# LiangZhaoPKUImperial/LinearSFM

Hardware: AMD Instinct MI355X
Metric: hierarchical linear map-joining solve wall-clock, NC3500-like stereo (all transforms + joins) (lower is better)
Workload: dtype f64

## Files before the change

### include/lsfm.h

```cpp
#ifndef LSFM_H
#define LSFM_H

#include <stddef.h>

#ifdef __cplusplus
extern "C" {
#endif

#define LSFM_OK 0
#define LSFM_ERR_ARG (-1)
#define LSFM_ERR_NO_DEVICE (-2)
#define LSFM_ERR_HIP (-3)
#define LSFM_ERR_OOM (-4)
#define LSFM_ERR_INTERNAL (-5)
#define LSFM_ERR_IO (-6)
#define LSFM_ERR_NOT_SPD (-7)
#define LSFM_NOT_CONVERGED 1

typedef struct lsfm_context lsfm_context;

typedef struct lsfm_map {
	int Ref, FRef, m, n, nU, nW;
	int ScaP, Fix, Sign, FScaP, FFix;
	int* stno;
// ... 170 lines not shown
int lsfm_save_pair_gate(const char* path, const int* ids, int K, const double* d2, const double* cov_diff);
int lsfm_read_pair_gate(const char* path, int* ids_f, int* ids_g, double* d2, double* cov_diff, int cap, int* count);
int lsfm_save_merge_report(const char* path, int K, int removed, int dof, double d2, const int* ids);
int lsfm_read_merge_report(const char* path, int* K, int* removed, int* dof, double* d2, int* ids, int cap);
int lsfm_save_state(const char* path, const double* st, const int* stno, int n);
int lsfm_save_state_bin(const char* path, const double* st, const int* stno, int n);
int lsfm_save_poses(const char* pose_path, const char* feat_path, const int* stno, const double* st, int n);

int lsfm_spmv_bench(lsfm_context* ctx, int m, const int* rowptr, const int* colidx, const double* val,
                    const double* x, double* y, int reps, double* avg_ms, double* algorithmic_bytes);

int lsfm_wstream_bench(lsfm_context* ctx, long long nblocks, int mode, int reps, double* avg_ms);

int lsfm_selftest_prims(lsfm_context* ctx, int cases, unsigned seed);

#define LSFM_SELFTEST_CHOL_INFO 16
int lsfm_selftest_chol(lsfm_context* ctx, int m, const int* rowptr, const int* colidx, const double* val, const int* origin, const unsigned char* fixed,
                       const int* pose_seg, int nseg, const double* r, int nrhs, int mode, double* z, double* dot, int* perm, int* colptr, int* rowidx,
                       double* L, double* Dinv, double* dscale, int cap_blocks, int* info);

int lsfm_selftest_transform(lsfm_context* ctx, const lsfm_map* maps, int N, int mono, const int* tref, const int* tscap, const int* tfix,
                            int alias_passthrough, lsfm_map* out);

int lsfm_selftest_small(lsfm_context* ctx, int G, const int* pose_off, const int* feat_off, const int* u_off, const unsigned char* active,
                        const double* U, const int* Ui, const int* Uj, const double* W, const int* photo, const int* feature, int nW, const double* V,
                        const double* ea, const double* eb, const double* x0, const unsigned char* fixed, int strips, double* x_pose, double* x_feat,
                        int* status, double* max_rel);

#ifdef __cplusplus
}
// ... 3 lines not shown
```

### linearsfm_amd/api.py

```python
from __future__ import annotations

import ctypes as C
import os

import numpy as np

_HERE = os.path.dirname(os.path.abspath(__file__))
LIB_PATH = os.path.join(_HERE, "liblsfm_hip.so")
_LIB = None

LSFM_OK = 0
LSFM_NOT_CONVERGED = 1


class LsfmMap(C.Structure):
    _fields_ = [("Ref", C.c_int), ("FRef", C.c_int), ("m", C.c_int), ("n", C.c_int), ("nU", C.c_int), ("nW", C.c_int),
                ("ScaP", C.c_int), ("Fix", C.c_int), ("Sign", C.c_int), ("FScaP", C.c_int), ("FFix", C.c_int),
                ("stno", C.POINTER(C.c_int)), ("stVal", C.POINTER(C.c_double)),
                ("U", C.POINTER(C.c_double)), ("Ui", C.POINTER(C.c_int)), ("Uj", C.POINTER(C.c_int)),
                ("W", C.POINTER(C.c_double)), ("photo", C.POINTER(C.c_int)), ("feature", C.POINTER(C.c_int)),
                ("V", C.POINTER(C.c_double)), ("FBlock", C.POINTER(C.c_int)), ("pose_origin", C.POINTER(C.c_int))]


class LsfmStats(C.Structure):
# ... 72 lines not shown
        L.lsfm_tree_free.argtypes = [vp, vp]
        L.lsfm_tree_free.restype = None
        L.lsfm_divide_conquer.argtypes = [vp, P(LsfmMap), C.c_int, C.c_int, P(LsfmMap), P(LsfmStats)]
        L.lsfm_read_localmap.argtypes = [C.c_char_p, C.c_int, P(LsfmMap)]
        L.lsfm_write_localmap.argtypes = [C.c_char_p, C.c_int, P(LsfmMap)]
        L.lsfm_read_localmaps.argtypes = [C.c_char_p, C.c_int, C.c_int, C.c_int, C.c_int, P(LsfmMap), P(C.c_int)]
        L.lsfm_write_mapset.argtypes = [C.c_char_p, P(LsfmMap), C.c_int, C.c_int]
        L.lsfm_mapset_info.argtypes = [C.c_char_p, P(C.c_int), P(C.c_int)]
        L.lsfm_read_mapset.argtypes = [C.c_char_p, C.c_int, C.c_int, C.c_int, C.c_int, P(LsfmMap)]
        L.lsfm_save_state_bin.argtypes = [C.c_char_p, P(C.c_double), P(C.c_int), C.c_int]
        L.lsfm_save_state.argtypes = [C.c_char_p, dp, ip, C.c_int]
        L.lsfm_save_poses.argtypes = [C.c_char_p, C.c_char_p, ip, dp, C.c_int]
        L.lsfm_schur_pattern.argtypes = [vp, ip, ip, ip, ip, C.c_int, C.c_int, C.c_int, C.c_int, ip, ip, C.c_int, ip]
        L.lsfm_symbolic_analyse.argtypes = [C.c_int, ip, ip, ip, C.c_int, ip, ip, ip, C.c_int, ip, dp]
        L.lsfm_inverse_v.argtypes = [vp, dp, C.c_int, C.c_int]
        L.lsfm_gn_polish.argtypes = [vp, P(LsfmMap), C.c_int, C.c_int, P(LsfmMap), C.c_int, dp, dp, ip]
        L.lsfm_gn_polish_robust.argtypes = [vp, P(LsfmMap), C.c_int, C.c_int, P(LsfmMap), C.c_int, C.c_int, C.c_double, dp, dp, ip, dp, dp]
        L.lsfm_map_chi2.argtypes = [vp, P(LsfmMap), C.c_int, C.c_int, P(LsfmMap), dp, ip]
        L.lsfm_map_feature_chi2.argtypes = [vp, P(LsfmMap), C.c_int, C.c_int, P(LsfmMap), dp, dp]
        L.lsfm_gn_polish_robust_features.argtypes = [vp, P(LsfmMap), C.c_int, C.c_int, P(LsfmMap), C.c_int, C.c_int, C.c_double, dp, dp, ip, dp, dp]
        L.lsfm_gn_linearise.argtypes = [vp, P(LsfmMap), C.c_int, C.c_int, P(LsfmMap), dp, P(LsfmMap), dp, dp]
        L.lsfm_gn_linearise_timed.argtypes = [vp, P(LsfmMap), C.c_int, C.c_int, P(LsfmMap), dp, P(LsfmMap), dp, dp, dp, ip]
        L.lsfm_solve_features.argtypes = [vp, dp, dp, dp, dp, dp, dp, C.c_int, C.c_int, ip, ip]
        L.lsfm_map_covariance.argtypes = [vp, P(LsfmMap), C.c_int, dp, dp, dp, C.c_int, ip]
        L.lsfm_map_covariance_timed.argtypes = [vp, P(LsfmMap), C.c_int, dp, dp, dp, C.c_int, ip, dp]
        L.lsfm_save_covariances.argtypes = [C.c_char_p, C.c_char_p, ip, C.c_int, C.c_int, dp, dp]
        L.lsfm_read_covariances.argtypes = [C.c_char_p, C.c_int, ip, dp, C.c_int, ip]
        L.lsfm_map_covariance_columns.argtypes = [vp, P(LsfmMap), C.c_int, ip, C.c_int, dp, dp, dp, ip, dp]
        L.lsfm_map_covariance_columns_timed.argtypes = [vp, P(LsfmMap), C.c_int, ip, C.c_int, dp, dp, dp, ip, dp, dp]
        L.lsfm_map_covariance_feature_columns.argtypes = [vp, P(LsfmMap), C.c_int, ip, C.c_int, dp, dp, dp, ip, dp]
# ... 26 lines not shown
        L.lsfm_selftest_chol.argtypes = [vp, C.c_int, ip, ip, dp, ip, P(C.c_ubyte), ip, C.c_int, dp, C.c_int, C.c_int, dp, dp, ip, ip, ip, dp, dp, dp,
                                         C.c_int, ip]
        L.lsfm_selftest_transform.argtypes = [vp, P(LsfmMap), C.c_int, C.c_int, ip, ip, ip, C.c_int, P(LsfmMap)]
        L.lsfm_selftest_small.argtypes = [vp, C.c_int, ip, ip, ip, ub, dp, ip, ip, dp, ip, ip, C.c_int, dp, dp, dp, dp, ub, C.c_int, dp, dp, ip, dp]
        _LIB = L
    return _LIB


EXPORTS = ["lsfm_context_create", "lsfm_context_destroy", "lsfm_set_pcg", "lsfm_set_precision", "lsfm_set_small_solve", "lsfm_set_spmv_variant", "lsfm_set_covcols_panel", "lsfm_last_error", "lsfm_stream",
           "lsfm_map_release", "lsfm_transform_stereo", "lsfm_transform_mono", "lsfm_join_stereo", "lsfm_join_mono",
           "lsfm_solve_stereo", "lsfm_solve_mono", "lsfm_tree_upload", "lsfm_tree_run", "lsfm_tree_set_final_reanchor",
           "lsfm_tree_download", "lsfm_tree_set_stop_level", "lsfm_tree_node_count", "lsfm_tree_download_node", "lsfm_tree_download_state", "lsfm_tree_set_plans", "lsfm_tree_export_size", "lsfm_tree_export_dev", "lsfm_packed_size",
           "lsfm_tree_upload_dev", "lsfm_tree_reload_dev", "lsfm_tree_set_comm", "lsfm_tree_set_comm_blocks", "lsfm_tree_export_slice_sizes", "lsfm_tree_export_slice_dev",
           "lsfm_tree_free", "lsfm_divide_conquer", "lsfm_read_localmap", "lsfm_read_localmaps", "lsfm_write_localmap", "lsfm_write_mapset", "lsfm_mapset_info", "lsfm_mapset_stamp", "lsfm_read_mapset", "lsfm_save_state_bin", "lsfm_save_state", "lsfm_save_poses", "lsfm_gn_polish",
           "lsfm_gn_polish_robust", "lsfm_map_chi2", "lsfm_map_feature_chi2", "lsfm_gn_polish_robust_features", "lsfm_gn_linearise", "lsfm_gn_linearise_timed",
           "lsfm_spmv_bench", "lsfm_wstream_bench", "lsfm_selftest_prims", "lsfm_selftest_chol", "lsfm_selftest_transform", "lsfm_selftest_small", "lsfm_schur_pattern", "lsfm_symbolic_analyse", "lsfm_inverse_v", "lsfm_solve_features",
           "lsfm_map_covariance", "lsfm_map_covariance_timed",
           "lsfm_save_covariances", "lsfm_read_covariances",
           "lsfm_map_covariance_columns", "lsfm_map_covariance_columns_timed", "lsfm_save_cov_columns", "lsfm_read_cov_columns",
           "lsfm_map_covariance_feature_columns", "lsfm_map_covariance_feature_columns_timed", "lsfm_map_feature_pair_gate", "lsfm_map_feature_pair_gate_timed", "lsfm_save_pair_gate", "lsfm_read_pair_gate",
           "lsfm_map_merge_features", "lsfm_map_merge_features_timed", "lsfm_merge_structure", "lsfm_save_merge_report", "lsfm_read_merge_report",
           "lsfm_map_marginalise", "lsfm_map_marginalise_timed", "lsfm_tree_export_reduced_size", "lsfm_tree_export_reduced_dev",
           "lsfm_tree_export_reduced_dev_timed", "lsfm_map_marginalise_poses", "lsfm_map_marginalise_poses_timed", "lsfm_marg_pose_structure", "lsfm_gn_structure"]


def _c(a, dtype):
    return np.ascontiguousarray(a, dtype=dtype).reshape(-1)


def _ptr(a, ctype):
    return a.ctypes.data_as(C.POINTER(ctype))
# ... 311 lines not shown
        t, cnt = np.zeros(3), np.zeros(4, np.int32)
        rc = lib().lsfm_gn_linearise_timed(self._h, arr, len(hms), int(mono), C.byref(x), _ptr(w, C.c_double) if w is not None else None,
                                           C.byref(out), C.byref(F), _ptr(b, C.c_double) if want_b else None,
                                           _ptr(t, C.c_double) if timed else None, _ptr(cnt, C.c_int) if timed else None)
        self._check(rc, "lsfm_gn_linearise")
        d = map_to_dict(out)
        if timed:
            return d, F.value, b, dict(zip(("assembly_ms", "coalesce_w_ms", "coalesce_u_ms"), t.tolist())), dict(zip(("NWJ", "nW", "NUJ", "nU"), cnt.tolist()))
        return d, F.value, b

    def inverse_v(self, V):
        IV = np.array(np.asarray(V, np.float64).reshape(-1), copy=True)
        n = IV.size // 9
        self._check(lib().lsfm_inverse_v(self._h, _ptr(IV, C.c_double), 0, n), "lsfm_inverse_v")
        return IV.reshape(n, 9)

    def solve_features(self, j, IV, eb, dpa):
        m, n = int(j["m"]), int(j["n"])
        W = _c(j["W"], np.float64); ph = _c(j["photo"], np.int32); fe = _c(j["feature"], np.int32)
        cnt = np.bincount(fe, minlength=n).astype(np.int32)
        IV = _c(IV, np.float64); eb = _c(eb, np.float64); dpa = _c(dpa, np.float64)
        dpb = np.zeros(3 * n)
        self._check(lib().lsfm_solve_features(self._h, _ptr(W, C.c_double), _ptr(IV, C.c_double), None, _ptr(eb, C.c_double), _ptr(dpa, C.c_double),
                                              _ptr(dpb, C.c_double), m, n, _ptr(cnt, C.c_int), _ptr(ph, C.c_int)), "lsfm_solve_features")
        return dpb

    def schur_pattern(self, j):
        m, n = int(j["m"]), int(j["n"])
        Ui = _c(j["Ui"], np.int32); Uj = _c(j["Uj"], np.int32); ph = _c(j["photo"], np.int32); fe = _c(j["feature"], np.int32)
        cap = m * (m + 1) // 2
# ... 526 lines not shown
```

### linearsfm_amd/csrc/lsfm_capi.hip

```cpp
#include <climits>
#include <cmath>
#include <cstring>

#include "lsfm_internal.hpp"
#include "lsfm_marg.hpp"
#include "lsfm_solve.hpp"
#include "lsfm_system.hpp"
#include "lsfm_tree.hpp"

using namespace lsfm;

namespace {

template <class F> int guarded(lsfm_context* ctx, F&& f)
{
	if (!ctx) return LSFM_ERR_ARG;
	struct Reset {
		lsfm_context* c;
		~Reset() { c->timed.clear(); c->ev_next = 0; c->plan = nullptr; }
	} reset{ ctx };
	try
	{
		if (hipSetDevice(ctx->device) != hipSuccess) return LSFM_ERR_NO_DEVICE;
		return f();
// ... 585 lines not shown
}

int lsfm_map_merge_features(lsfm_context* ctx, const lsfm_map* map, int mono, const int* pairs, int K, lsfm_map* out, double* d2, int* dof, int* rep,
                            int* steps, double* last_corr)
{
	return lsfm_map_merge_features_timed(ctx, map, mono, pairs, K, out, d2, dof, rep, steps, last_corr, nullptr);
}

int lsfm_inverse_v(lsfm_context* ctx, double* V, int m, int n)
{
	(void)m;
	if (n < 0 || (n && !V)) return LSFM_ERR_ARG;
	return guarded(ctx, [&]() { return inverse_v(ctx, V, n); });
}

int lsfm_solve_features(lsfm_context* ctx, const double* W, const double* IV, const double* ea, const double* eb, const double* dpa, double* dpb,
                        int m, int n, const int* mapCor, const int* photo)
{
	(void)ea;
	if (m <= 0 || n < 0 || !dpa || (n && (!W || !IV || !eb || !dpb || !mapCor || !photo))) return LSFM_ERR_ARG;
	return guarded(ctx, [&]() { return solve_features(ctx, W, IV, eb, dpa, dpb, m, n, mapCor, photo); });
}

int lsfm_schur_pattern(lsfm_context* ctx, const int* Ui, const int* Uj, const int* photo, const int* feature, int m, int n, int nU, int nW, int* rowptr,
                       int* colidx, int cap, int* nnzb)
{
	if (m <= 0 || n < 0 || nU < 0 || nW < 0 || !rowptr || !colidx || !nnzb || (nU && (!Ui || !Uj)) || (nW && (!photo || !feature))) return LSFM_ERR_ARG;
	return guarded(ctx, [&]() {
		HostSystem h;
		h.m = m; h.n = n; h.nU = nU; h.nW = nW;
// ... 107 lines not shown
```

### linearsfm_amd/csrc/lsfm_device.hpp

```cpp
#pragma once
#include <hip/hip_runtime.h>

#define LSFM_WAVE 64
#define LSFM_PI_REF 3.1415926

namespace lsfm {

__device__ __forceinline__ bool tr_stereo_hub(int pose_id, int tref) { return tref >= 0 && pose_id == tref; }
__device__ __forceinline__ bool tr_keeps_u(int a, int b, int h0, int h1) { return a != h0 && b != h0 && a != h1 && b != h1; }
__device__ __forceinline__ bool tr_keeps_w(int k, int h0, int h1) { return k != h0 && k != h1; }

template <int N>
__device__ __forceinline__ void ld(double* dst, const double* __restrict__ src)
{
#pragma unroll
	for (int i = 0; i < N; i++) dst[i] = src[i];
}
template <int N>
__device__ __forceinline__ void ld(double* dst, const float* __restrict__ src)
{
#pragma unroll
	for (int i = 0; i < N; i++) dst[i] = (double)src[i];
}
template <int N>
// ... 159 lines not shown
	for (int off = 32; off > 0; off >>= 1) v += __shfl_xor(v, off, LSFM_WAVE);
	return v;
}
template <int LANES>
__device__ __forceinline__ double block_sum_fixed(double v, double* part)
{
	v = wave_sum(v);
	if ((threadIdx.x & (LSFM_WAVE - 1)) == 0) part[threadIdx.x / LSFM_WAVE] = v;
	__syncthreads();
	double sum = 0.0;
#pragma unroll
	for (int w = 0; w < LANES / LSFM_WAVE; w++) sum += part[w];
	return sum;
}

__device__ __forceinline__ void atomic_add_f64(double* p, double v)
{
	__hip_atomic_fetch_add(p, v, __ATOMIC_RELAXED, __HIP_MEMORY_SCOPE_AGENT);
}

__device__ __forceinline__ void atomic_add_i64(long long* p, long long v)
{
	__hip_atomic_fetch_add(reinterpret_cast<unsigned long long*>(p), (unsigned long long)v, __ATOMIC_RELAXED, __HIP_MEMORY_SCOPE_AGENT);
}
__device__ __forceinline__ void lds_add_i64(long long* p, long long v)
{
	__hip_atomic_fetch_add(reinterpret_cast<unsigned long long*>(p), (unsigned long long)v, __ATOMIC_RELAXED, __HIP_MEMORY_SCOPE_WORKGROUP);
}
__device__ __forceinline__ long long to_fixed(double v, int sh, bool& bad)
{
// ... 105 lines not shown
	if (!valid) return;
	const int sl = lds_slot(keys, cap, key);
#pragma unroll
	for (int i = 0; i < N; i++) stage[i] = x[i];
	const int rot = (threadIdx.x & (LSFM_WAVE - 1)) % N;
#pragma unroll 1
	for (int e = 0; e < N; e++)
	{
		int i = e + rot;
		if (i >= N) i -= N;
		const double v = stage[i];
		if (sl >= 0) lds_add_f64(vals + sl * N + i, v); else atomic_add_f64(gdst + i, v);
	}
}
template <int N>
__device__ __forceinline__ void tile_clear(int* keys, double* vals, int cap)
{
	for (int i = threadIdx.x; i < cap; i += blockDim.x) keys[i] = -1;
	for (int i = threadIdx.x; i < cap * N; i += blockDim.x) vals[i] = 0.0;
}
template <int N>
__device__ __forceinline__ void tile_flush(const int* keys, const double* vals, int cap, double* gbase)
{
	for (int i = threadIdx.x; i < cap * N; i += blockDim.x)
	{
		const int k = keys[i / N];
		if (k >= 0) atomic_add_f64(gbase + (size_t)k * N + i % N, vals[i]);
	}
}

template <int TW, class EntryFn, class FeatFn>
__device__ __forceinline__ void tile_runs(int nft, const int* sFp, double* sT, EntryFn entry, FeatFn feat)
{
	const int tid = threadIdx.x, nt = blockDim.x;
	int la = 0;
	while (la < nft)
	{
		const int e0 = sFp[la];
		int lo = la + 1, hi = nft;
		while (lo < hi) { const int mid = (lo + hi + 1) >> 1; if (sFp[mid] - e0 <= nt) lo = mid; else hi = mid - 1; }
		const int lb = lo, e1 = sFp[lb];
		for (int ce0 = e0;; ce0 += nt)
		{
// ... 26 lines not shown
```

### linearsfm_amd/csrc/lsfm_internal.hpp

```cpp
#pragma once
#include <hip/hip_runtime.h>

#include <cstdint>
#include <cstdio>
#include <condition_variable>
#include <cstring>
#include <exception>
#include <functional>
#include <memory>
#include <mutex>
#include <thread>
#include <string>
#include <vector>

#include "../../include/lsfm.h"
#include "lsfm_map.hpp"

namespace lsfm {

struct Error { int code; std::string msg; };
struct DevBatch;
struct IndexHold;
struct SolvePlan;
struct PreLevel;
// ... 379 lines not shown
                       int* halvings, double* fchi2, double* fweight);
int map_chi2(lsfm_context* ctx, const lsfm_map* maps, int N, bool mono, const lsfm_map* x, double* chi2, int* dof);
int gn_linearise(lsfm_context* ctx, const lsfm_map* maps, int N, bool mono, const lsfm_map* x, const double* weight, lsfm_map* out, double* obj,
                 double* b, double* times, int* counts);
int map_covariance(lsfm_context* ctx, const lsfm_map* map, bool mono, double* pose_cov, double* feat_cov, double* pair_cov, int cap_blocks, int* nnzb,
                   double* times);
int map_covariance_columns(lsfm_context* ctx, const lsfm_map* map, bool mono, const int* poses, int k, double* pose_cols, double* feat_cols, double* joint,
                           int* steps, double* last_corr, double* times);
int map_covariance_feature_columns(lsfm_context* ctx, const lsfm_map* map, bool mono, const int* feats, int k, double* pose_cols, double* feat_cols,
                                   double* joint, int* steps, double* last_corr, double* times);
int map_feature_pair_gate(lsfm_context* ctx, const lsfm_map* map, bool mono, const int* pairs, int K, double* d2, double* cov_diff, int* steps,
                          double* last_corr, double* times);
int map_merge_features(lsfm_context* ctx, const lsfm_map* map, bool mono, const int* pairs, int K, lsfm_map* out, double* d2, int* dof, int* rep,
                       int* steps, double* last_corr, double* times);
int inverse_v(lsfm_context* ctx, double* V, int n);
int solve_features(lsfm_context* ctx, const double* W, const double* IV, const double* eb, const double* dpa, double* dpb, int m, int n, const int* mapCor,
                   const int* photo);
bool no_timing_events();
#define LSFM_REC_T(e, s) do { if (!lsfm::no_timing_events()) LSFM_CHECK_HIP(hipEventRecord(e, s)); } while (0)
unsigned timing_event_flags();
unsigned order_event_flags();
void prefetch_next_level(lsfm_context* ctx, const DevBatch& Y, const std::vector<int>& target_ref, int next_level, int step_hint,
                         const unsigned long long* level_keys, int level_nnzb);
int spmv_external(lsfm_context* ctx, int m, const int* rowptr, const int* colidx, const double* val, const double* x, double* y, int reps,
                  double* avg_ms, double* bytes);
int chol_selftest(lsfm_context* ctx, int m, const int* rowptr, const int* colidx, const double* val, const int* origin, const unsigned char* fixed,
                  const int* pose_seg, int nseg, const double* r, int nrhs, int mode, double* z, double* dot, int* perm, int* colptr, int* rowidx,
                  double* L, double* Dinv, double* dscale, int cap_blocks, int* info);

int wstream_bench(lsfm_context* ctx, long long nblocks, int mode, int reps, double* avg_ms);
// ... 3 lines not shown
```

### linearsfm_amd/csrc/lsfm_solve.hip

```cpp
#include <algorithm>
#include <cmath>

#include "lsfm_device.hpp"
#include "lsfm_internal.hpp"
#include "lsfm_solve.hpp"

namespace lsfm {

__global__ void __launch_bounds__(256) k_vinv(int NF, const double* __restrict__ V, const double* __restrict__ eb, double* __restrict__ IV, double* __restrict__ LY,
                                               double* __restrict__ ymax, RhsFused rhs, double* __restrict__ uu)
{
	__shared__ double wmax[4];
	int f = blockIdx.x * blockDim.x + threadIdx.x;
	double y2 = 0.0;
	if (f < NF)
	{
	double a[9], o[9];
	ld<9>(a, V + (size_t)f * 9);
	inv3_sym(a, o);
	st<9>(IV + (size_t)f * 9, o);
	const double* e = eb + (size_t)f * 3;
	double l[9];
	const double d0 = o[0];
	l[0] = sqrt(d0);
	l[1] = o[3] / l[0];
	l[3] = o[6] / l[0];
	const double d1 = o[4] - l[1] * l[1];
	l[2] = sqrt(d1);
	l[4] = (o[7] - l[3] * l[1]) / l[2];
	const double d2 = o[8] - l[3] * l[3] - l[4] * l[4];
	l[5] = sqrt(d2);
	l[6] = l[0] * e[0] + l[1] * e[1] + l[3] * e[2];
	l[7] = l[2] * e[1] + l[4] * e[2];
	l[8] = l[5] * e[2];
	if (!(d0 > 0.0) || !(d1 > 0.0) || !(d2 > 0.0)) l[0] = __builtin_nan("");
	st<9>(LY + (size_t)f * 9, l);
	y2 = l[6] * l[6] + l[7] * l[7] + l[8] * l[8];
	if (uu)
	{
#pragma unroll
		for (int sd = 0; sd < 2; sd++)
		{
			const int fs = sd ? rhs.srcC[f] : rhs.srcE[f];
			double u0 = 0.0, u1 = 0.0, u2 = 0.0;
			if (fs >= 0)
			{
				const double* x = rhs.feat_src + (size_t)fs * 3;
				u0 = x[0] / l[0];
				u1 = (x[1] - l[1] * u0) / l[2];
				u2 = (x[2] - l[3] * u0 - l[4] * u1) / l[5];
			}
			uu[(size_t)f * 6 + 3 * sd] = u0; uu[(size_t)f * 6 + 3 * sd + 1] = u1; uu[(size_t)f * 6 + 3 * sd + 2] = u2;
			y2 = fmax(y2, u0 * u0 + u1 * u1 + u2 * u2);
		}
	}
	if (!(y2 == y2)) y2 = 0.0;
	}
	if (!ymax) return;
#pragma unroll
	for (int off = 32; off > 0; off >>= 1) y2 = fmax(y2, __shfl_xor(y2, off, LSFM_WAVE));
	if ((threadIdx.x & (LSFM_WAVE - 1)) == 0) wmax[threadIdx.x >> 6] = y2;
	__syncthreads();
	if (threadIdx.x == 0) ymax[blockIdx.x] = fmax(fmax(wmax[0], wmax[1]), fmax(wmax[2], wmax[3]));
}

__device__ __forceinline__ int half_exponent(double d)
{
	if (!(d > 0.0) || !(d < 1e300)) return 0;
	int k;
	(void)frexp(d, &k);
	return ((k + 1) >> 1) + 1;
}
// ... 652 lines not shown
{
	ctx->ensure_arenas((size_t)n * 400 + ((size_t)64 << 20));
	ctx->arena[0].reset(); ctx->scratch.reset();
	double* dV = ctx->arena[0].alloc<double>((size_t)n * 9);
	double* dIV = ctx->arena[0].alloc<double>((size_t)n * 9);
	h2d(ctx, dV, V, (size_t)n * 9 * sizeof(double));
	if (n)
	{
		double* LY = ctx->scratch.alloc<double>((size_t)n * 9);
		double* eb = ctx->scratch.alloc<double>((size_t)n * 3);
		dev_zero(ctx, eb, (size_t)n * 3 * sizeof(double));
		hipLaunchKernelGGL(k_vinv, dim3((n + 255) / 256), dim3(256), 0, ctx->stream, n, dV, eb, dIV, LY, (double*)nullptr, RhsFused(), (double*)nullptr);
		LSFM_CHECK_HIP(hipStreamSynchronize(ctx->stream));
	}
	d2h(ctx, V, dIV, (size_t)n * 9 * sizeof(double));
	return LSFM_OK;
}
int solve_features(lsfm_context* ctx, const double* W, const double* IV, const double* eb, const double* dpa, double* dpb, int m, int n, const int* mapCor,
                   const int* photo)
{
	std::vector<int> fptr((size_t)n + 1, 0);
	for (int f = 0; f < n; f++)
	{
		if (mapCor[f] < 0) LSFM_FAIL(LSFM_ERR_ARG, "negative block count of a feature");
		fptr[f + 1] = fptr[f] + mapCor[f];
	}
	const int nW = fptr[n];
	for (int j = 0; j < nW; j++) if (photo[j] < 0 || photo[j] >= m) LSFM_FAIL(LSFM_ERR_ARG, "photo index out of range");
	ctx->ensure_arenas((size_t)nW * 200 + (size_t)n * 300 + (size_t)m * 100 + ((size_t)64 << 20));
	ctx->arena[0].reset(); ctx->scratch.reset();
// ... 56 lines not shown
```

### linearsfm_amd/csrc/lsfm_transform.hip

```cpp
#include <algorithm>
#include <climits>
#include <cstddef>

#include "lsfm_device.hpp"
#include "lsfm_internal.hpp"

namespace lsfm {

struct TMap {
	int active, nh;
	int P0, m, F0, n;
	int U0, U0n, W0, W0n, kU0, kW0;
	int hub[2];
	int nref, nscap;
	int newFix, oldFix, newLabel;
	int c2fix, c3zero;
	int tref, tscap, oldref, oldscap;
	double R1[9], t1[3], scale1;
	int sign1;
	double R[9], dRA[9], dRB[9], dRG[9], t[3], dA[3], dB[3], dG[3];
	double Scale, Scale2, dSdA[3], dSdB[3], dSdG[3], dSdt[9], dSdtt[9];
};

__global__ void k_tr_find(const int* __restrict__ pose_id, const int* __restrict__ pose_map, int M, TMap* tm)
// ... 258 lines not shown

__global__ void k_tr_gather_counts(const int* __restrict__ KU, const int* __restrict__ KW, const int* __restrict__ uoff, const int* __restrict__ woff,
                                   int B, int* __restrict__ out, const TMap* __restrict__ tm, const int* __restrict__ err)
{
	int b = blockIdx.x * blockDim.x + threadIdx.x;
	if (b > B) return;
	out[b] = KU[uoff[b]];
	out[B + 1 + b] = KW[woff[b]];
	if (b < B) out[2 * (B + 1) + b] = tm[b].active > 0 ? tm[b].sign1 : 0;
	else out[2 * (B + 1) + B] = *err;
}

#define TRE_TILE 128
#define TRE_ROUND 256
#define TRE_MAPS 4
#define TR_REC 39
static_assert(offsetof(TMap, dRA) == offsetof(TMap, R) + 72 && offsetof(TMap, dRB) == offsetof(TMap, R) + 144 && offsetof(TMap, dRG) == offsetof(TMap, R) + 216 &&
              offsetof(TMap, t) == offsetof(TMap, R) + 288, "R, dRA, dRB, dRG, t of TMap are read as one run of TR_REC doubles");

__device__ __forceinline__ void stereo_tf(const double* rec, const double* xn, double* Tf)
{
	double dd[3] = { xn[0] - rec[36], xn[1] - rec[37], xn[2] - rec[38] }, tmp1[3], tmp2[3], tmp3[3];
	mv3(rec + 9, dd, tmp1); mv3(rec + 18, dd, tmp2); mv3(rec + 27, dd, tmp3);
#pragma unroll
	for (int r = 0; r < 3; r++) { Tf[3 * r] = tmp1[r]; Tf[3 * r + 1] = tmp2[r]; Tf[3 * r + 2] = tmp3[r]; }
}

template <int NH>
__global__ void __launch_bounds__(256)
k_tr_feat_pre(int NF, const TMap* __restrict__ tm, const int* __restrict__ feat_map, const double* __restrict__ feat, const int* __restrict__ fptr,
              const double* __restrict__ Vold, const int* __restrict__ KW, double* __restrict__ nfeat, int* __restrict__ nfptr,
              double* __restrict__ Vn, double* __restrict__ FD, int4* __restrict__ finfo, int* __restrict__ hubJ)
{
	const int f = blockIdx.x * blockDim.x + threadIdx.x;
	if (f >= NF) return;
#pragma unroll
	for (int sidx = 0; sidx < NH; sidx++) hubJ[(size_t)f * NH + sidx] = -1;
	const TMap* t = &tm[feat_map[f]];
	const int j0 = fptr[f];
	const double* x = feat + (size_t)f * 3;
	if (!(t->active > 0 && t->nh == NH))
	{
		nfeat[3 * (size_t)f] = x[0]; nfeat[3 * (size_t)f + 1] = x[1]; nfeat[3 * (size_t)f + 2] = x[2];
		for (int i = 0; i < 9; i++) Vn[(size_t)f * 9 + i] = Vold[(size_t)f * 9 + i];
		nfptr[f] = t->W0n + (j0 - t->W0);
		finfo[f] = make_int4(0, -1, NH == 2 ? -1 : feat_map[f], -j0);
		return;
	}
	nfptr[f] = t->W0n + NH * (f - t->F0) + (KW[j0] - t->kW0);
	finfo[f] = make_int4(1, t->hub[0], NH == 2 ? t->hub[1] : feat_map[f], NH - KW[j0]);
	double Df[9], Cf[NH][18], xn[3];
	double d[3] = { x[0] - t->t1[0], x[1] - t->t1[1], x[2] - t->t1[2] };
	mv3(t->R1, d, xn);
	if (NH == 2) { xn[0] = xn[0] / t->scale1; xn[1] = xn[1] / t->scale1; xn[2] = xn[2] / t->scale1; }
	nfeat[3 * (size_t)f] = xn[0]; nfeat[3 * (size_t)f + 1] = xn[1]; nfeat[3 * (size_t)f + 2] = xn[2];
	if constexpr (NH == 1)
	{
		ld<9>(Df, t->R);
	}
	else
	{
		double adt[9], atmp[9], adtt[9];
		mono_trans_jac(*t, xn, Df, adt, atmp, adtt);
#pragma unroll
		for (int r = 0; r < 3; r++)
		{
#pragma unroll
			for (int c = 0; c < 3; c++) { Cf[0][6 * r + c] = adt[3 * r + c]; Cf[NH - 1][6 * r + c] = adtt[3 * r + c]; Cf[NH - 1][6 * r + 3 + c] = 0.0; }
			Cf[0][6 * r + 3] = atmp[3 * r]; Cf[0][6 * r + 4] = atmp[3 * r + 1]; Cf[0][6 * r + 5] = atmp[3 * r + 2];
		}
		if (t->c2fix)
#pragma unroll
			for (int r = 0; r < 3; r++)
#pragma unroll
				for (int c = 0; c < 6; c++)
					if (c == t->newFix) Cf[0][6 * r + c] = 0.0;
		if (t->c3zero) zero<18>(Cf[NH - 1]);
	}
	double V[9], T[9], Vnew[9];
	ld<9>(V, Vold + (size_t)f * 9);
	mtm<3, 3, 3, false>(Df, V, T);
	mm<3, 3, 3, false>(T, Df, Vnew);
	st<9>(Vn + (size_t)f * 9, Vnew);
	if constexpr (NH == 2)
	{
		double* fd = FD + (size_t)f * (9 + 18 * NH);
		st<9>(fd, Df);
#pragma unroll
		for (int s = 0; s < NH; s++) st<18>(fd + 9 + 18 * s, Cf[s]);
	}
}

#ifdef LSFM_K9_TIMING
__device__ unsigned long long g_tr_t[16];
#define TRT_DECL unsigned long long tracc[12] = { 0, 0, 0, 0, 0, 0, 0, 0, 0, 0, 0, 0 }; unsigned long long trprev = __builtin_readcyclecounter()
#define TRT(i) do { const unsigned long long n_ = __builtin_readcyclecounter(); tracc[i] += n_ - trprev; trprev = n_; } while (0)
#define TRT_FLUSH() do { if (threadIdx.x == 0) { for (int i_ = 0; i_ < 12; i_++) atomicAdd(&g_tr_t[i_], tracc[i_]); atomicAdd(&g_tr_t[12], 1ull); } } while (0)
extern "C" void lsfm_debug_tr(unsigned long long* out, int reset)
{
	(void)hipDeviceSynchronize();
	if (out) (void)hipMemcpyFromSymbol(out, HIP_SYMBOL(g_tr_t), sizeof(unsigned long long) * 16);
	if (reset) { unsigned long long z[16] = { 0 }; (void)hipMemcpyToSymbol(HIP_SYMBOL(g_tr_t), z, sizeof(z)); }
}
#else
#define TRT_DECL do { } while (0)
// ... 288 lines not shown
#pragma unroll
	for (int s = 0; s < NH; s++) tile_flush<36>(gkeys, gvals + s * GCAP * 36, GCAP, Gpose + (size_t)s * M * 36);
	TRT(9);
	TRT_FLUSH();
}

template <int NH>
__global__ void __launch_bounds__(256, NH == 1 ? 2 : 1)
k_tr_feat_post(int NF, int M, const TMap* __restrict__ tm, const int* __restrict__ feat_map, const int* __restrict__ fptr,
               const double* __restrict__ Vold, const double* __restrict__ Wold, const int* __restrict__ photo, const double* __restrict__ Dp,
               const double* __restrict__ FD, const double* __restrict__ xnew, const double* __restrict__ Gsum, const int* __restrict__ hubJ,
               const int* __restrict__ wbase, const int* __restrict__ newf, int* __restrict__ srcf, double* __restrict__ Wn_,
               int* __restrict__ nphoto, int* __restrict__ nfeature, double* __restrict__ PP)
{
	constexpr int TW = 18 * NH;
	const int f = blockIdx.x * blockDim.x + threadIdx.x;
	const bool inb = f < NF;
	const TMap* t = inb ? &tm[feat_map[f]] : nullptr;
	const bool act = inb && t->active > 0 && t->nh == NH;
	double Df[9], Cf[NH][18], G[NH][18];
	if (act)
	{
		const double* fd = NH == 2 ? FD + (size_t)f * (9 + TW) : nullptr;
		if constexpr (NH == 1) ld<9>(Df, t->R); else ld<9>(Df, fd);
		const int base = wbase[f];
		const int hubs[2] = { t->hub[0], NH == 2 ? t->hub[1] : -1 };
		double hubW[NH][18];
#pragma unroll
		for (int s = 0; s < NH; s++) zero<18>(hubW[s]);
		bool walk = false;
// ... 54 lines not shown
			mtm<3, 6, 3, true>(G[s], Df, Wh);
			st<18>(Wn_ + (size_t)(base + s) * 18, Wh);
			nphoto[base + s] = hubs[s]; nfeature[base + s] = newf ? newf[f] : f;
			if (srcf) srcf[base + s] = f;
		}
	}
#pragma unroll
	for (int s = 0; s < NH; s++)
#pragma unroll
		for (int s2 = s; s2 < NH; s2++)
		{
			double P[36];
			if (act) mtm<3, 6, 6, false>(Cf[s], G[s2], P);
			const int idx = (s == 0 ? s2 : 2);
			const int mp = act ? feat_map[f] : 0;
			wave_scatter_add<36>(PP + ((size_t)mp * 3 + idx) * 36, P, act);
		}
}

template <int NH>
__global__ void __launch_bounds__(128, 1)
k_tr_ublocks(int NU, int M, const TMap* __restrict__ tm, const int* __restrict__ pose_map, const double* __restrict__ Uold,
             const int* __restrict__ Ui, const int* __restrict__ Uj, const int* __restrict__ KU, const double* __restrict__ Dp,
             const double* __restrict__ Cp, double* __restrict__ Un, int* __restrict__ nUi, int* __restrict__ nUj,
             double* __restrict__ Gpose)
{
	constexpr int GCAP = 64;
	__shared__ int gkeys[GCAP];
	__shared__ double gvals[NH * GCAP * 36];
	__shared__ double sStage[128 * 37];
	for (int q = threadIdx.x; q < GCAP; q += blockDim.x) gkeys[q] = -1;
	for (int q = threadIdx.x; q < NH * GCAP * 36; q += blockDim.x) gvals[q] = 0.0;
// ... 65 lines not shown
}

__device__ __forceinline__ void add_oriented(double* dst, const double* X, int r, int c)
{
	if (r < c) { for (int q = 0; q < 36; q++) dst[q] += X[q]; }
	else if (r > c) { for (int i = 0; i < 6; i++) for (int j = 0; j < 6; j++) dst[j * 6 + i] += X[i * 6 + j]; }
	else { for (int i = 0; i < 6; i++) for (int j = 0; j < 6; j++) dst[i * 6 + j] += X[i * 6 + j] + X[j * 6 + i]; }
}

template <int NH>
__global__ void __launch_bounds__(128, 1)
k_tr_poseslots(int M, const TMap* __restrict__ tm, const int* __restrict__ pose_map, const double* __restrict__ Dp,
                               const double* __restrict__ Cp, const double* __restrict__ Gpose, double* __restrict__ Un, int* __restrict__ nUi,
                               int* __restrict__ nUj, double* __restrict__ PP)
{
	const int k0 = blockIdx.x * blockDim.x + threadIdx.x;
	const bool inb = k0 < M;
	const int k = inb ? k0 : 0;
	const int mp = pose_map[k];
	const TMap& t = tm[mp];
	const bool act = inb && t.active > 0 && t.nh == NH;
	double D[36];
	ld<36>(D, Dp + (size_t)k * 36);
	const int h0 = t.hub[0], h1 = NH == 2 ? t.hub[1] : -1;
	const int slot1 = t.U0n + (k - t.P0), slot2 = t.U0n + t.m + (k - t.P0);
	if (act)
	{
		if (k <= h0) { nUi[slot1] = k; nUj[slot1] = h0; } else { nUi[slot1] = h0; nUj[slot1] = k; }
		if (NH == 2) { if (k <= h0) { nUi[slot2] = k; nUj[slot2] = h1; } else { nUi[slot2] = h1; nUj[slot2] = k; } }
	}
// ... 11 lines not shown
			if (h0 < h1) { for (int q = 0; q < 36; q++) atomic_add_f64(dst + q, X[q]); }
			else { for (int i = 0; i < 6; i++) for (int j = 0; j < 6; j++) atomic_add_f64(dst + j * 6 + i, X[i * 6 + j]); }
		}
		else if (NH == 2 && s == 0 && k == h1)
		{
			double* dst = Un + (size_t)slot1 * 36;
			if (h1 < h0) { for (int q = 0; q < 36; q++) atomic_add_f64(dst + q, X[q]); }
			else { for (int i = 0; i < 6; i++) for (int j = 0; j < 6; j++) atomic_add_f64(dst + j * 6 + i, X[i * 6 + j]); }
		}
		else
		{
			double* dst = Un + (size_t)(s == 0 ? slot1 : slot2) * 36;
			add_oriented(dst, X, k, hs);
		}
#pragma unroll
		for (int s0 = 0; s0 <= s; s0++)
		{
			double C[36], P[36];
			ld<36>(C, Cp + (size_t)s0 * M * 36 + (size_t)k * 36);
			mtm<6, 6, 6, false>(C, G, P);
			const int idx = (s0 == 0 ? s : 2);
			wave_scatter_add<36>(PP + ((size_t)mp * 3 + idx) * 36, P, act);
		}
	}
}

template <int NH>
__global__ void k_tr_diag(int B, const TMap* __restrict__ tm, const double* __restrict__ PP, double* __restrict__ Un)
{
	int b = blockIdx.x * blockDim.x + threadIdx.x;
	if (b >= B) return;
	const TMap& t = tm[b];
	if (t.active <= 0 || t.nh != NH) return;
	const double* P = PP + (size_t)b * 3 * 36;
	double* d0 = Un + (size_t)(t.U0n + (t.hub[0] - t.P0)) * 36;
	for (int q = 0; q < 36; q++) d0[q] += P[q];
	if (NH == 2)
	{
		double* d2 = Un + (size_t)(t.U0n + t.m + (t.hub[1] - t.P0)) * 36;
// ... 301 lines not shown
```

Before: 30.52.

## Stage strided feature records through LDS and tile per-map projection accumulation

Routes the per-feature 9- and 3-double records in k_vinv and k_tr_feat_pre through shared-memory tiles, so global loads and stores become coalesced double2 accesses instead of strided per-thread ones. Replaces wave_scatter_add on the per-map PP accumulators with a new wave-level segmented reduction into a small LDS hash tile, flushed once per block, to cut global f64 atomics. The cost is more shared memory, extra barriers, and a wave shuffle reduction tree. A self-test entry point for the inverse-V kernel is also added.

```diff
diff --git a/include/lsfm.h b/include/lsfm.h
--- a/include/lsfm.h
+++ b/include/lsfm.h
@@ -208,6 +208,8 @@
 
 int lsfm_selftest_prims(lsfm_context* ctx, int cases, unsigned seed);
 
+int lsfm_selftest_vinv(lsfm_context* ctx, const double* V, const double* eb, int n, int skip, double* IV, double* LY);
+
 #define LSFM_SELFTEST_CHOL_INFO 16
 int lsfm_selftest_chol(lsfm_context* ctx, int m, const int* rowptr, const int* colidx, const double* val, const int* origin, const unsigned char* fixed,
                        const int* pose_seg, int nseg, const double* r, int nrhs, int mode, double* z, double* dot, int* perm, int* colptr, int* rowidx,
diff --git a/linearsfm_amd/api.py b/linearsfm_amd/api.py
--- a/linearsfm_amd/api.py
+++ b/linearsfm_amd/api.py
@@ -110,6 +110,7 @@
         L.lsfm_schur_pattern.argtypes = [vp, ip, ip, ip, ip, C.c_int, C.c_int, C.c_int, C.c_int, ip, ip, C.c_int, ip]
         L.lsfm_symbolic_analyse.argtypes = [C.c_int, ip, ip, ip, C.c_int, ip, ip, ip, C.c_int, ip, dp]
         L.lsfm_inverse_v.argtypes = [vp, dp, C.c_int, C.c_int]
+        L.lsfm_selftest_vinv.argtypes = [vp, dp, dp, C.c_int, C.c_int, dp, dp]
         L.lsfm_gn_polish.argtypes = [vp, P(LsfmMap), C.c_int, C.c_int, P(LsfmMap), C.c_int, dp, dp, ip]
         L.lsfm_gn_polish_robust.argtypes = [vp, P(LsfmMap), C.c_int, C.c_int, P(LsfmMap), C.c_int, C.c_int, C.c_double, dp, dp, ip, dp, dp]
         L.lsfm_map_chi2.argtypes = [vp, P(LsfmMap), C.c_int, C.c_int, P(LsfmMap), dp, ip]
@@ -166,7 +167,7 @@
            "lsfm_tree_upload_dev", "lsfm_tree_reload_dev", "lsfm_tree_set_comm", "lsfm_tree_set_comm_blocks", "lsfm_tree_export_slice_sizes", "lsfm_tree_export_slice_dev",
            "lsfm_tree_free", "lsfm_divide_conquer", "lsfm_read_localmap", "lsfm_read_localmaps", "lsfm_write_localmap", "lsfm_write_mapset", "lsfm_mapset_info", "lsfm_mapset_stamp", "lsfm_read_mapset", "lsfm_save_state_bin", "lsfm_save_state", "lsfm_save_poses", "lsfm_gn_polish",
            "lsfm_gn_polish_robust", "lsfm_map_chi2", "lsfm_map_feature_chi2", "lsfm_gn_polish_robust_features", "lsfm_gn_linearise", "lsfm_gn_linearise_timed",
-           "lsfm_spmv_bench", "lsfm_wstream_bench", "lsfm_selftest_prims", "lsfm_selftest_chol", "lsfm_selftest_transform", "lsfm_selftest_small", "lsfm_schur_pattern", "lsfm_symbolic_analyse", "lsfm_inverse_v", "lsfm_solve_features",
+           "lsfm_spmv_bench", "lsfm_wstream_bench", "lsfm_selftest_prims", "lsfm_selftest_chol", "lsfm_selftest_transform", "lsfm_selftest_small", "lsfm_schur_pattern", "lsfm_symbolic_analyse", "lsfm_inverse_v", "lsfm_selftest_vinv", "lsfm_solve_features",
            "lsfm_map_covariance", "lsfm_map_covariance_timed",
            "lsfm_save_covariances", "lsfm_read_covariances",
            "lsfm_map_covariance_columns", "lsfm_map_covariance_columns_timed", "lsfm_save_cov_columns", "lsfm_read_cov_columns",
@@ -508,6 +509,16 @@
         n = IV.size // 9
         self._check(lib().lsfm_inverse_v(self._h, _ptr(IV, C.c_double), 0, n), "lsfm_inverse_v")
         return IV.reshape(n, 9)
+
+    def selftest_vinv(self, V, eb, skip=0):
+        V = _c(np.asarray(V, np.float64).reshape(-1), np.float64); eb = _c(np.asarray(eb, np.float64).reshape(-1), np.float64)
+        n = V.size // 9
+        if V.size != 9 * n or eb.size != 3 * n:
+            raise LsfmError("selftest_vinv: V [n, 9] and eb [n, 3]")
+        IV = np.zeros(9 * n); LY = np.zeros(9 * n)
+        self._check(lib().lsfm_selftest_vinv(self._h, _ptr(V, C.c_double), _ptr(eb, C.c_double), n, int(skip), _ptr(IV, C.c_double), _ptr(LY, C.c_double)),
+                    "lsfm_selftest_vinv")
+        return IV.reshape(n, 9), LY.reshape(n, 9)
 
     def solve_features(self, j, IV, eb, dpa):
         m, n = int(j["m"]), int(j["n"])
diff --git a/linearsfm_amd/csrc/lsfm_capi.hip b/linearsfm_amd/csrc/lsfm_capi.hip
--- a/linearsfm_amd/csrc/lsfm_capi.hip
+++ b/linearsfm_amd/csrc/lsfm_capi.hip
@@ -623,6 +623,12 @@
 	return guarded(ctx, [&]() { return inverse_v(ctx, V, n); });
 }
 
+int lsfm_selftest_vinv(lsfm_context* ctx, const double* V, const double* eb, int n, int skip, double* IV, double* LY)
+{
+	if (n < 0 || skip < 0 || skip > 1 || (n && (!V || !eb || !IV || !LY))) return LSFM_ERR_ARG;
+	return guarded(ctx, [&]() { return vinv_selftest(ctx, V, eb, n, skip, IV, LY); });
+}
+
 int lsfm_solve_features(lsfm_context* ctx, const double* W, const double* IV, const double* ea, const double* eb, const double* dpa, double* dpb,
                         int m, int n, const int* mapCor, const int* photo)
 {
diff --git a/linearsfm_amd/csrc/lsfm_device.hpp b/linearsfm_amd/csrc/lsfm_device.hpp
--- a/linearsfm_amd/csrc/lsfm_device.hpp
+++ b/linearsfm_amd/csrc/lsfm_device.hpp
@@ -197,6 +197,38 @@
 	return sum;
 }
 
+template <int S, int OFF>
+__device__ __forceinline__ double wave_sum_spread(const double* v, bool on, int lane)
+{
+	if constexpr (OFF == 0) return on ? v[0] : 0.0;
+	else
+	{
+		constexpr int H = (S + 1) / 2;
+		const bool up = (lane & OFF) != 0;
+		double w[H];
+#pragma unroll
+		for (int i = 0; i < H; i++)
+		{
+			const double lo = on ? v[i] : 0.0, hi = (i + H < S && on) ? v[i + H < S ? i + H : 0] : 0.0;
+			w[i] = (up ? hi : lo) + __shfl_xor(up ? lo : hi, OFF, LSFM_WAVE);
+		}
+		return wave_sum_spread<H, OFF / 2>(w, true, lane);
+	}
+}
+template <int S>
+__device__ __forceinline__ int wave_spread_index(int lane)
+{
+	int off = 0, len = S, s = S;
+#pragma unroll
+	for (int o = LSFM_WAVE / 2; o; o >>= 1)
+	{
+		const int h = (s + 1) / 2;
+		if (lane & o) { off += h; len -= h; } else len = min(len, h);
+		s = h;
+	}
+	return len >= 1 ? off : -1;
+}
+
 __device__ __forceinline__ void atomic_add_f64(double* p, double v)
 {
 	__hip_atomic_fetch_add(p, v, __ATOMIC_RELAXED, __HIP_MEMORY_SCOPE_AGENT);
@@ -332,6 +364,39 @@
 	}
 }
 template <int N>
+__device__ __forceinline__ void tile_wave_add(int* keys, double* vals, int cap, int key, double* gbase, const double* x, bool valid)
+{
+	static_assert(N <= LSFM_WAVE, "one lane per value");
+	unsigned long long todo = __ballot(valid), alone = 0ull;
+	if (todo == 0ull) return;
+	const int lane = threadIdx.x & (LSFM_WAVE - 1), mine = wave_spread_index<N>(lane);
+#pragma unroll 1
+	for (int round = 0; round < 4 && todo; round++)
+	{
+		const int leader = __ffsll((long long)todo) - 1;
+		const int first = __shfl(key, leader, LSFM_WAVE);
+		const bool same = valid && key == first;
+		const unsigned long long grp = __ballot(same);
+		if (__popcll(grp) > 1)
+		{
+			const double keep = wave_sum_spread<N, LSFM_WAVE / 2>(x, same, lane);
+			int sl = -1;
+			if (lane == leader) sl = lds_slot(keys, cap, first);
+			sl = __shfl(sl, leader, LSFM_WAVE);
+			if (mine >= 0) { if (sl >= 0) lds_add_f64(vals + sl * N + mine, keep); else atomic_add_f64(gbase + (size_t)first * N + mine, keep); }
+		}
+		else alone |= grp;
+		todo &= ~grp;
+	}
+	alone |= todo;
+	if (valid && ((alone >> lane) & 1ull))
+	{
+		const int sl = lds_slot(keys, cap, key);
+#pragma unroll
+		for (int i = 0; i < N; i++) { if (sl >= 0) lds_add_f64(vals + sl * N + i, x[i]); else atomic_add_f64(gbase + (size_t)key * N + i, x[i]); }
+	}
+}
+template <int N>
 __device__ __forceinline__ void tile_clear(int* keys, double* vals, int cap)
 {
 	for (int i = threadIdx.x; i < cap; i += blockDim.x) keys[i] = -1;
@@ -345,6 +410,38 @@
 		const int k = keys[i / N];
 		if (k >= 0) atomic_add_f64(gbase + (size_t)k * N + i % N, vals[i]);
 	}
+}
+
+template <int N>
+__device__ __forceinline__ void tile_records_load(double* tile, const double* __restrict__ g, int nrec)
+{
+	static_assert(N % 2 == 1, "an even record length needs a padded stride in the tile");
+	const int len = nrec * N, head = (int)(((size_t)g >> 3) & 1);
+	if (len <= 0) return;
+	if (threadIdx.x == 0 && head) tile[0] = g[0];
+	const int pairs = (len - head) >> 1;
+	for (int p = threadIdx.x; p < pairs; p += blockDim.x)
+	{
+		const int j = head + 2 * p;
+		const double2 v = *reinterpret_cast<const double2*>(g + j);
+		tile[j] = v.x; tile[j + 1] = v.y;
+	}
+	if (threadIdx.x == 0 && ((len - head) & 1)) tile[len - 1] = g[len - 1];
+}
+template <int N>
+__device__ __forceinline__ void tile_records_store(const double* tile, double* __restrict__ g, int nrec)
+{
+	static_assert(N % 2 == 1, "an even record length needs a padded stride in the tile");
+	const int len = nrec * N, head = (int)(((size_t)g >> 3) & 1);
+	if (len <= 0) return;
+	if (threadIdx.x == 0 && head) g[0] = tile[0];
+	const int pairs = (len - head) >> 1;
+	for (int p = threadIdx.x; p < pairs; p += blockDim.x)
+	{
+		const int j = head + 2 * p;
+		*reinterpret_cast<double2*>(g + j) = make_double2(tile[j], tile[j + 1]);
+	}
+	if (threadIdx.x == 0 && ((len - head) & 1)) g[len - 1] = tile[len - 1];
 }
 
 template <int TW, class EntryFn, class FeatFn>
diff --git a/linearsfm_amd/csrc/lsfm_internal.hpp b/linearsfm_amd/csrc/lsfm_internal.hpp
--- a/linearsfm_amd/csrc/lsfm_internal.hpp
+++ b/linearsfm_amd/csrc/lsfm_internal.hpp
@@ -417,6 +417,7 @@
 int map_merge_features(lsfm_context* ctx, const lsfm_map* map, bool mono, const int* pairs, int K, lsfm_map* out, double* d2, int* dof, int* rep,
                        int* steps, double* last_corr, double* times);
 int inverse_v(lsfm_context* ctx, double* V, int n);
+int vinv_selftest(lsfm_context* ctx, const double* V, const double* eb, int n, int skip, double* IV, double* LY);
 int solve_features(lsfm_context* ctx, const double* W, const double* IV, const double* eb, const double* dpa, double* dpb, int m, int n, const int* mapCor,
                    const int* photo);
 bool no_timing_events();
diff --git a/linearsfm_amd/csrc/lsfm_solve.hip b/linearsfm_amd/csrc/lsfm_solve.hip
--- a/linearsfm_amd/csrc/lsfm_solve.hip
+++ b/linearsfm_amd/csrc/lsfm_solve.hip
@@ -11,16 +11,22 @@
                                                double* __restrict__ ymax, RhsFused rhs, double* __restrict__ uu)
 {
 	__shared__ double wmax[4];
-	int f = blockIdx.x * blockDim.x + threadIdx.x;
+	__shared__ double sRec[256 * 9], sEb[256 * 3];
+	const int f0 = blockIdx.x * 256, nrec = min(256, NF - f0);
+	int f = f0 + threadIdx.x;
+	tile_records_load<9>(sRec, V + (size_t)f0 * 9, nrec);
+	tile_records_load<3>(sEb, eb + (size_t)f0 * 3, nrec);
+	__syncthreads();
 	double y2 = 0.0;
+	double* rec = sRec + threadIdx.x * 9;
+	double l[9];
 	if (f < NF)
 	{
 	double a[9], o[9];
-	ld<9>(a, V + (size_t)f * 9);
+	ld<9>(a, rec);
 	inv3_sym(a, o);
-	st<9>(IV + (size_t)f * 9, o);
-	const double* e = eb + (size_t)f * 3;
-	double l[9];
+	st<9>(rec, o);
+	const double* e = sEb + threadIdx.x * 3;
 	const double d0 = o[0];
 	l[0] = sqrt(d0);
 	l[1] = o[3] / l[0];
@@ -34,7 +40,6 @@
 	l[7] = l[2] * e[1] + l[4] * e[2];
 	l[8] = l[5] * e[2];
 	if (!(d0 > 0.0) || !(d1 > 0.0) || !(d2 > 0.0)) l[0] = __builtin_nan("");
-	st<9>(LY + (size_t)f * 9, l);
 	y2 = l[6] * l[6] + l[7] * l[7] + l[8] * l[8];
 	if (uu)
 	{
@@ -56,6 +61,12 @@
 	}
 	if (!(y2 == y2)) y2 = 0.0;
 	}
+	__syncthreads();
+	tile_records_store<9>(sRec, IV + (size_t)f0 * 9, nrec);
+	__syncthreads();
+	if (f < NF) st<9>(rec, l);
+	__syncthreads();
+	tile_records_store<9>(sRec, LY + (size_t)f0 * 9, nrec);
 	if (!ymax) return;
 #pragma unroll
 	for (int off = 32; off > 0; off >>= 1) y2 = fmax(y2, __shfl_xor(y2, off, LSFM_WAVE));
@@ -738,6 +749,24 @@
 		LSFM_CHECK_HIP(hipStreamSynchronize(ctx->stream));
 	}
 	d2h(ctx, V, dIV, (size_t)n * 9 * sizeof(double));
+	return LSFM_OK;
+}
+int vinv_selftest(lsfm_context* ctx, const double* V, const double* eb, int n, int skip, double* IV, double* LY)
+{
+	ctx->ensure_arenas((size_t)n * 400 + ((size_t)64 << 20));
+	ctx->arena[0].reset(); ctx->scratch.reset();
+	Arena& ar = ctx->arena[0];
+	double* dV = ar.alloc<double>((size_t)n * 9 + skip) + skip;
+	double* deb = ar.alloc<double>((size_t)n * 3 + skip) + skip;
+	double* dIV = ar.alloc<double>((size_t)n * 9 + skip) + skip;
+	double* dLY = ar.alloc<double>((size_t)n * 9 + skip) + skip;
+	if (!n) return LSFM_OK;
+	h2d(ctx, dV, V, (size_t)n * 9 * sizeof(double));
+	h2d(ctx, deb, eb, (size_t)n * 3 * sizeof(double));
+	hipLaunchKernelGGL(k_vinv, dim3((n + 255) / 256), dim3(256), 0, ctx->stream, n, dV, deb, dIV, dLY, (double*)nullptr, RhsFused(), (double*)nullptr);
+	LSFM_CHECK_HIP(hipStreamSynchronize(ctx->stream));
+	d2h(ctx, IV, dIV, (size_t)n * 9 * sizeof(double));
+	d2h(ctx, LY, dLY, (size_t)n * 9 * sizeof(double));
 	return LSFM_OK;
 }
 int solve_features(lsfm_context* ctx, const double* W, const double* IV, const double* eb, const double* dpa, double* dpb, int m, int n, const int* mapCor,
diff --git a/linearsfm_amd/csrc/lsfm_transform.hip b/linearsfm_amd/csrc/lsfm_transform.hip
--- a/linearsfm_amd/csrc/lsfm_transform.hip
+++ b/linearsfm_amd/csrc/lsfm_transform.hip
@@ -296,6 +296,7 @@
 #define TRE_TILE 128
 #define TRE_ROUND 256
 #define TRE_MAPS 4
+#define TR_PCAP(NH) ((NH) == 1 ? 4 : 16)
 #define TR_REC 39
 static_assert(offsetof(TMap, dRA) == offsetof(TMap, R) + 72 && offsetof(TMap, dRB) == offsetof(TMap, R) + 144 && offsetof(TMap, dRG) == offsetof(TMap, R) + 216 &&
               offsetof(TMap, t) == offsetof(TMap, R) + 288, "R, dRA, dRB, dRG, t of TMap are read as one run of TR_REC doubles");
@@ -309,22 +310,16 @@
 }
 
 template <int NH>
-__global__ void __launch_bounds__(256)
-k_tr_feat_pre(int NF, const TMap* __restrict__ tm, const int* __restrict__ feat_map, const double* __restrict__ feat, const int* __restrict__ fptr,
-              const double* __restrict__ Vold, const int* __restrict__ KW, double* __restrict__ nfeat, int* __restrict__ nfptr,
-              double* __restrict__ Vn, double* __restrict__ FD, int4* __restrict__ finfo, int* __restrict__ hubJ)
-{
-	const int f = blockIdx.x * blockDim.x + threadIdx.x;
-	if (f >= NF) return;
+__device__ __forceinline__ void feat_pre_lane(int f, const TMap* __restrict__ tm, const int* __restrict__ feat_map, const int* __restrict__ fptr,
+                                              const int* __restrict__ KW, int* __restrict__ nfptr, double* __restrict__ FD, int4* __restrict__ finfo,
+                                              int* __restrict__ hubJ, double* x, double* v)
+{
 #pragma unroll
 	for (int sidx = 0; sidx < NH; sidx++) hubJ[(size_t)f * NH + sidx] = -1;
 	const TMap* t = &tm[feat_map[f]];
 	const int j0 = fptr[f];
-	const double* x = feat + (size_t)f * 3;
 	if (!(t->active > 0 && t->nh == NH))
 	{
-		nfeat[3 * (size_t)f] = x[0]; nfeat[3 * (size_t)f + 1] = x[1]; nfeat[3 * (size_t)f + 2] = x[2];
-		for (int i = 0; i < 9; i++) Vn[(size_t)f * 9 + i] = Vold[(size_t)f * 9 + i];
 		nfptr[f] = t->W0n + (j0 - t->W0);
 		finfo[f] = make_int4(0, -1, NH == 2 ? -1 : feat_map[f], -j0);
 		return;
@@ -335,7 +330,7 @@
 	double d[3] = { x[0] - t->t1[0], x[1] - t->t1[1], x[2] - t->t1[2] };
 	mv3(t->R1, d, xn);
 	if (NH == 2) { xn[0] = xn[0] / t->scale1; xn[1] = xn[1] / t->scale1; xn[2] = xn[2] / t->scale1; }
-	nfeat[3 * (size_t)f] = xn[0]; nfeat[3 * (size_t)f + 1] = xn[1]; nfeat[3 * (size_t)f + 2] = xn[2];
+	x[0] = xn[0]; x[1] = xn[1]; x[2] = xn[2];
 	if constexpr (NH == 1)
 	{
 		ld<9>(Df, t->R);
@@ -360,10 +355,10 @@
 		if (t->c3zero) zero<18>(Cf[NH - 1]);
 	}
 	double V[9], T[9], Vnew[9];
-	ld<9>(V, Vold + (size_t)f * 9);
+	ld<9>(V, v);
 	mtm<3, 3, 3, false>(Df, V, T);
 	mm<3, 3, 3, false>(T, Df, Vnew);
-	st<9>(Vn + (size_t)f * 9, Vnew);
+	st<9>(v, Vnew);
 	if constexpr (NH == 2)
 	{
 		double* fd = FD + (size_t)f * (9 + 18 * NH);
@@ -371,6 +366,23 @@
 #pragma unroll
 		for (int s = 0; s < NH; s++) st<18>(fd + 9 + 18 * s, Cf[s]);
 	}
+}
+
+template <int NH>
+__global__ void __launch_bounds__(256)
+k_tr_feat_pre(int NF, const TMap* __restrict__ tm, const int* __restrict__ feat_map, const double* __restrict__ feat, const int* __restrict__ fptr,
+              const double* __restrict__ Vold, const int* __restrict__ KW, double* __restrict__ nfeat, int* __restrict__ nfptr,
+              double* __restrict__ Vn, double* __restrict__ FD, int4* __restrict__ finfo, int* __restrict__ hubJ)
+{
+	__shared__ double sV[256 * 9], sX[256 * 3];
+	const int f0 = blockIdx.x * 256, nrec = min(256, NF - f0), f = f0 + threadIdx.x;
+	tile_records_load<9>(sV, Vold + (size_t)f0 * 9, nrec);
+	tile_records_load<3>(sX, feat + (size_t)f0 * 3, nrec);
+	__syncthreads();
+	if (f < NF) feat_pre_lane<NH>(f, tm, feat_map, fptr, KW, nfptr, FD, finfo, hubJ, sX + threadIdx.x * 3, sV + threadIdx.x * 9);
+	__syncthreads();
+	tile_records_store<9>(sV, Vn + (size_t)f0 * 9, nrec);
+	tile_records_store<3>(sX, nfeat + (size_t)f0 * 3, nrec);
 }
 
 #ifdef LSFM_K9_TIMING
@@ -689,6 +701,10 @@
                int* __restrict__ nphoto, int* __restrict__ nfeature, double* __restrict__ PP)
 {
 	constexpr int TW = 18 * NH;
+	__shared__ int pkeys[TR_PCAP(NH)];
+	__shared__ double pvals[TR_PCAP(NH) * 36];
+	tile_clear<36>(pkeys, pvals, TR_PCAP(NH));
+	__syncthreads();
 	const int f = blockIdx.x * blockDim.x + threadIdx.x;
 	const bool inb = f < NF;
 	const TMap* t = inb ? &tm[feat_map[f]] : nullptr;
@@ -773,8 +789,10 @@
 			if (act) mtm<3, 6, 6, false>(Cf[s], G[s2], P);
 			const int idx = (s == 0 ? s2 : 2);
 			const int mp = act ? feat_map[f] : 0;
-			wave_scatter_add<36>(PP + ((size_t)mp * 3 + idx) * 36, P, act);
-		}
+			tile_wave_add<36>(pkeys, pvals, TR_PCAP(NH), mp * 3 + idx, PP, P, act);
+		}
+	__syncthreads();
+	tile_flush<36>(pkeys, pvals, TR_PCAP(NH), PP);
 }
 
 template <int NH>
@@ -870,6 +888,10 @@
                                const double* __restrict__ Cp, const double* __restrict__ Gpose, double* __restrict__ Un, int* __restrict__ nUi,
                                int* __restrict__ nUj, double* __restrict__ PP)
 {
+	__shared__ int pkeys[TR_PCAP(NH)];
+	__shared__ double pvals[TR_PCAP(NH) * 36];
+	tile_clear<36>(pkeys, pvals, TR_PCAP(NH));
+	__syncthreads();
 	const int k0 = blockIdx.x * blockDim.x + threadIdx.x;
 	const bool inb = k0 < M;
 	const int k = inb ? k0 : 0;
@@ -911,15 +933,18 @@
 			add_oriented(dst, X, k, hs);
 		}
 #pragma unroll
-		for (int s0 = 0; s0 <= s; s0++)
-		{
+		for (int s0 = 0; s0 < NH; s0++)
+		{
+			if (s0 > s) continue;
 			double C[36], P[36];
 			ld<36>(C, Cp + (size_t)s0 * M * 36 + (size_t)k * 36);
 			mtm<6, 6, 6, false>(C, G, P);
 			const int idx = (s0 == 0 ? s : 2);
-			wave_scatter_add<36>(PP + ((size_t)mp * 3 + idx) * 36, P, act);
-		}
-	}
+			tile_wave_add<36>(pkeys, pvals, TR_PCAP(NH), mp * 3 + idx, PP, P, act);
+		}
+	}
+	__syncthreads();
+	tile_flush<36>(pkeys, pvals, TR_PCAP(NH), PP);
 }
 
 template <int NH>
```

Measured after the change: 30.05, median of 6. 1.02x faster.
